# tinganchen/AlignQ

Hardware: AMD Instinct MI355X
Metric: images/sec (train step, CDF+ADMM) ResNet-20 8-bit (higher is better)
Workload: dtype f32; 1 GPU; resnet20 CIFAR-shape 3x32x32, 8W/8A CDF+ADMM full train step (cdf_alignment_admm/resnet-20-cifar-10), batch 128/GPU, HIP-graph replay, batch-norm folded into the site kernels, channels-last tensors, all Conv2d_Q convolutions on alignq_conv*_nhwc (exact-product bf16 MFMA); global_batch=128, parallelism=dp1

## Files before the change

alignq_amd/csrc/conv_kernels.hip:

```cpp
#include <hip/hip_runtime.h>
#include <stdint.h>
#include <stdlib.h>

#include "../../include/alignq.h"
#include "site_internal.h"
#include "wgrad_reduce_body.h"

namespace {

using namespace alignq_wgr;

typedef __bf16 bf16x8 __attribute__((ext_vector_type(8)));
typedef __bf16 bf16x4 __attribute__((ext_vector_type(4)));
typedef float f32x4 __attribute__((ext_vector_type(4)));
typedef short s16x4 __attribute__((ext_vector_type(4)));

__device__ __forceinline__ s16x4 tr_read(const __bf16* p) {
  return __builtin_amdgcn_ds_read_tr16_b64_v4i16((__attribute__((address_space(3))) s16x4*)(p));
}
__device__ __forceinline__ bf16x8 join8(s16x4 a, s16x4 b) {
  typedef short s16x8 __attribute__((ext_vector_type(8)));
  s16x8 v = {a[0], a[1], a[2], a[3], b[0], b[1], b[2], b[3]};
  return __builtin_bit_cast(bf16x8, v);
}


template <int xb>
__device__ __forceinline__ f32x4 fetch_act4(const float* __restrict__ x, int64_t off) {
  if constexpr (xb == 0) return *reinterpret_cast<const f32x4*>(x + off);
  if constexpr (xb == 2) {
    const s16x4 b = *reinterpret_cast<const s16x4*>(reinterpret_cast<const short*>(x) + off);
    return (f32x4){(float)b[0], (float)b[1], (float)b[2], (float)b[3]};
  }
  const char4 b = *reinterpret_cast<const char4*>(reinterpret_cast<const signed char*>(x) + off);
  return (f32x4){(float)b.x, (float)b.y, (float)b.z, (float)b.w};
}

struct BnLazy {
  const float* z;
  const float* ab;
  const float* save;
  const float* ktot;
  const float* part = nullptr;
  int n_tiles = 0, tile_f = 0;
  double inv_n = 1.0;
  float* dgamma = nullptr;
  float* dbeta = nullptr;
};

template <int C>
__device__ __forceinline__ void bn_totals_lds(const BnLazy& t, float* __restrict__ kt, bool publish) {
  static_assert(256 % C == 0, "thread -> (channel, group)");
  __shared__ double red[256][2];
  constexpr int G = 256 / C;
  const int tid = threadIdx.x;
  const int cp = C < t.tile_f ? C : t.tile_f;
  const int cyc = C / cp, cnt = t.n_tiles / cyc;
  const int c = tid % C, grp = tid / C;
  const int e = c % cp, t_first = c / cp;
  double s0 = 0, s1 = 0;
  constexpr int U = 16;
  for (int i0 = grp; i0 < cnt; i0 += G * U) {
    float2 v[U];
#pragma unroll
    for (int u = 0; u < U; u++) {
      const int i = i0 + u * G;
      const int ic = i < cnt ? i : cnt - 1;
      v[u] = *reinterpret_cast<const float2*>(t.part + ((int64_t)(ic * cyc + t_first) * cp + e) * 2);
// ... 11 lines not shown
#pragma unroll
    for (int g = 0; g < G; g++) { t0 += red[g * C + tid][0]; t1 += red[g * C + tid][1]; }
    kt[tid] = (float)(t0 * t.inv_n);
    kt[C + tid] = (float)(t1 * t.inv_n);
    if (publish) {
      if (t.dbeta) t.dbeta[tid] = (float)t0;
      if (t.dgamma) t.dgamma[tid] = (float)t1;
    }
  }
  __syncthreads();
}

__device__ __forceinline__ float4 bn_lazy4(const float4& g, const float4& z, const float4& a, const float4& m, const float4& is,
                                           const float4& k0, const float4& k1) {
  float4 o;
  o.x = a.x * (g.x - k0.x - (z.x - m.x) * is.x * k1.x);
  o.y = a.y * (g.y - k0.y - (z.y - m.y) * is.y * k1.y);
  o.z = a.z * (g.z - k0.z - (z.z - m.z) * is.z * k1.z);
  o.w = a.w * (g.w - k0.w - (z.w - m.w) * is.w * k1.w);
  return o;
}

template <int C> constexpr int conv_cp() { return C == 16 ? 16 : (C == 32 ? 48 : C + 8); }
template <int C, int WD, int PT>
struct ConvLds {
  static constexpr int kBf16 = 3 * ((PT / WD) + 2) * (WD + 2) * conv_cp<C>();
};

template <int C, int WD, int PT, bool DGRAD, int XB = 0>
__device__ __forceinline__ void conv3x3_body(const float* __restrict__ x, const float* __restrict__ w,
                                             float* __restrict__ y, int H, int total_rows, float nlev, __bf16* lds,
                                             int block, const float* __restrict__ add,
                                             float* __restrict__ bn_part = nullptr, int n_wg = 0,
                                             BnLazy lazy = BnLazy{nullptr, nullptr, nullptr, nullptr}, float xlev = 1.0f) {
  static_assert(XB == 0 || !DGRAD, "the data gradient reads fp32 dy");
  constexpr int xb = XB;
  constexpr int TR = PT / WD;
  constexpr int NS = (9 * C + 31) / 32;
  constexpr int NCG = C / 16;
  constexpr int NPP = 4 / NCG;
  constexpr int NG = PT / 16;
  constexpr int LW = WD + 2;
  constexpr int CP = conv_cp<C>();
  constexpr int LROWS = TR + 2;
  constexpr int ARR = LROWS * LW * CP;
  static_assert(3 * ARR == ConvLds<C, WD, PT>::kBf16, "LDS size");
  __bf16* Xhi = lds;
  __bf16* Xmi = lds + ARR;
  __bf16* Xlo = lds + 2 * ARR;

  const int tid = threadIdx.x, lane = tid & 63, wv = tid >> 6;
  const int row0 = block * TR;
  const int img_lo = (row0 / H) * H, img_hi = img_lo + H;
  {
    constexpr int C4 = C / 4;
    constexpr int N4 = LROWS * LW * C4;
    constexpr int NIT = (N4 + 255) / 256;
    float4 v[NIT];
#pragma unroll
    for (int it = 0; it < NIT; it++) {
      const int i = tid + 256 * it;
      const int c4 = i % C4, col = (i / C4) % LW, lr = i / (C4 * LW);
      const int grow = row0 + lr - 1;
      const bool ok = i < N4 && col >= 1 && col <= WD && grow >= img_lo && grow < img_hi && grow < total_rows;
      const int64_t off = ok ? ((int64_t)grow * WD + (col - 1)) * C + 4 * c4 : 0;
      const f32x4 ld = fetch_act4<XB>(x, off);
      v[it] = ok ? make_float4(ld[0], ld[1], ld[2], ld[3]) : make_float4(0.f, 0.f, 0.f, 0.f);
    }
    if (DGRAD && lazy.z) {
      float4 zz[NIT];
#pragma unroll
      for (int it = 0; it < NIT; it++) {
        const int i = tid + 256 * it;
        const int c4 = i % C4, col = (i / C4) % LW, lr = i / (C4 * LW);
        const int grow = row0 + lr - 1;
        const bool ok = i < N4 && col >= 1 && col <= WD && grow >= img_lo && grow < img_hi && grow < total_rows;
        zz[it] = *reinterpret_cast<const float4*>(lazy.z + (ok ? ((int64_t)grow * WD + (col - 1)) * C + 4 * c4 : 0));
      }
      const int c4t = tid % C4;
      const float4 a4 = *reinterpret_cast<const float4*>(lazy.ab + 4 * c4t);
      const float4 m4 = *reinterpret_cast<const float4*>(lazy.save + 4 * c4t);
      const float4 i4 = *reinterpret_cast<const float4*>(lazy.save + C + 4 * c4t);
      float4 k0, k1;
      if (lazy.part) {
        __shared__ __attribute__((aligned(16))) float kt[2 * C];
        bn_totals_lds<C>(lazy, kt, block == 0);
        k0 = *reinterpret_cast<const float4*>(kt + 4 * c4t);
        k1 = *reinterpret_cast<const float4*>(kt + C + 4 * c4t);
      } else {
        k0 = *reinterpret_cast<const float4*>(lazy.ktot + 4 * c4t);
        k1 = *reinterpret_cast<const float4*>(lazy.ktot + C + 4 * c4t);
      }
#pragma unroll
      for (int it = 0; it < NIT; it++) {
        const int i = tid + 256 * it;
        const int col = (i / C4) % LW, lr = i / (C4 * LW);
        const int grow = row0 + lr - 1;
        const bool ok = i < N4 && col >= 1 && col <= WD && grow >= img_lo && grow < img_hi && grow < total_rows;
        if (ok) v[it] = bn_lazy4(v[it], zz[it], a4, m4, i4, k0, k1);
      }
    }
#pragma unroll
    for (int it = 0; it < NIT; it++) {
      const int i = tid + 256 * it;
      if (i < N4) {
        const int c4 = i % C4, col = (i / C4) % LW, lr = i / (C4 * LW);
        bf16x4 h4, m4, l4;
        const float vv[4] = {v[it].x, v[it].y, v[it].z, v[it].w};
#pragma unroll
        for (int e = 0; e < 4; e++) {
          const __bf16 hi = (__bf16)vv[e];
          const float r1 = vv[e] - (float)hi;
          const __bf16 mi = (__bf16)r1;
          const float r2 = r1 - (float)mi;
          h4[e] = hi; m4[e] = mi; l4[e] = (__bf16)r2;
        }
        const int o = (lr * LW + col) * CP + 4 * c4;
        *reinterpret_cast<bf16x4*>(Xhi + o) = h4;
        *reinterpret_cast<bf16x4*>(Xmi + o) = m4;
        *reinterpret_cast<bf16x4*>(Xlo + o) = l4;
      }
    }
  }
  const int cog = wv % NCG, pp = wv / NCG;
  const int m = lane & 15, q = lane >> 4;
  bf16x8 ab[NS];
#pragma unroll
  for (int s = 0; s < NS; s++) {
    const int k0 = 32 * s + 8 * q;
    const int tap = k0 / C, c0 = k0 % C;
    float v[8];
    if (tap < 9) {
      if (!DGRAD) {
        const float* p = w + ((int64_t)(cog * 16 + m) * 9 + tap) * C + c0;
        const float4 a4 = *reinterpret_cast<const float4*>(p), b4 = *reinterpret_cast<const float4*>(p + 4);
        v[0] = a4.x; v[1] = a4.y; v[2] = a4.z; v[3] = a4.w; v[4] = b4.x; v[5] = b4.y; v[6] = b4.z; v[7] = b4.w;
      } else {
#pragma unroll
        for (int j = 0; j < 8; j++) v[j] = w[((int64_t)(c0 + j) * 9 + (8 - tap)) * C + cog * 16 + m];
      }
    } else {
#pragma unroll
      for (int j = 0; j < 8; j++) v[j] = 0.f;
    }
#pragma unroll
    for (int j = 0; j < 8; j++) ab[s][j] = (__bf16)rintf(v[j] * nlev);
  }
  __syncthreads();
  float bs[4] = {0.f, 0.f, 0.f, 0.f}, bq[4] = {0.f, 0.f, 0.f, 0.f};
  for (int g = pp; g < NG; g += NPP) {
    const int p = g * 16 + (lane & 15);
    const int r = p / WD, c = p % WD;
    f32x4 acc = {0.f, 0.f, 0.f, 0.f};
#pragma unroll
    for (int s = 0; s < NS; s++) {
      const int k0 = 32 * s + 8 * q;
      const int tap = k0 / C, c0 = k0 % C;
      bf16x8 bh, bm, bl;
      if (tap < 9) {
        const int ky = tap / 3, kx = tap % 3;
        const int o = ((r + ky) * LW + (c + kx)) * CP + c0;
        bh = *reinterpret_cast<const bf16x8*>(Xhi + o);
        bm = *reinterpret_cast<const bf16x8*>(Xmi + o);
        bl = *reinterpret_cast<const bf16x8*>(Xlo + o);
      } else {
#pragma unroll
        for (int j = 0; j < 8; j++) { bh[j] = (__bf16)0.f; bm[j] = (__bf16)0.f; bl[j] = (__bf16)0.f; }
      }
      if (DGRAD || xb == 0) acc = __builtin_amdgcn_mfma_f32_16x16x32_bf16(ab[s], bl, acc, 0, 0, 0);
      acc = __builtin_amdgcn_mfma_f32_16x16x32_bf16(ab[s], bm, acc, 0, 0, 0);
      acc = __builtin_amdgcn_mfma_f32_16x16x32_bf16(ab[s], bh, acc, 0, 0, 0);
    }
    const int grow = row0 + r;
    if (grow < total_rows) {
      const int64_t o = ((int64_t)grow * WD + c) * C + cog * 16 + 4 * q;
      const float den = (!DGRAD && xb != 0) ? nlev * xlev : nlev;
      float4 v = make_float4(acc[0] / den, acc[1] / den, acc[2] / den, acc[3] / den);
      if (add) {
        const float4 r = *reinterpret_cast<const float4*>(add + o);
        v.x += r.x; v.y += r.y; v.z += r.z; v.w += r.w;
      }
      *reinterpret_cast<float4*>(y + o) = v;
      bs[0] += v.x; bs[1] += v.y; bs[2] += v.z; bs[3] += v.w;
      bq[0] += v.x * v.x; bq[1] += v.y * v.y; bq[2] += v.z * v.z; bq[3] += v.w * v.w;
    }
  }
  if (!DGRAD && bn_part) {
    float* red = reinterpret_cast<float*>(lds);
#define ROW_SHR_ADD(V, CTRL) V += __builtin_bit_cast(float, __builtin_amdgcn_update_dpp(0, __builtin_bit_cast(int, V), CTRL, 0xf, 0xf, false))
#pragma unroll
    for (int e = 0; e < 4; e++) {
      ROW_SHR_ADD(bs[e], 0x111); ROW_SHR_ADD(bs[e], 0x112); ROW_SHR_ADD(bs[e], 0x114); ROW_SHR_ADD(bs[e], 0x118);
      ROW_SHR_ADD(bq[e], 0x111); ROW_SHR_ADD(bq[e], 0x112); ROW_SHR_ADD(bq[e], 0x114); ROW_SHR_ADD(bq[e], 0x118);
    }
#undef ROW_SHR_ADD
    __syncthreads();
    if ((lane & 15) == 15) {
#pragma unroll
      for (int e = 0; e < 4; e++) {
        red[(wv * 16 + 4 * q + e) * 2] = bs[e];
        red[(wv * 16 + 4 * q + e) * 2 + 1] = bq[e];
      }
    }
    __syncthreads();
    if (tid < C) {
      const int cg = tid / 16, cl = tid % 16;
      float s0 = 0.f, s1 = 0.f;
#pragma unroll
      for (int ppi = 0; ppi < NPP; ppi++) {
        const int w2 = ppi * NCG + cg;
        s0 += red[(w2 * 16 + cl) * 2];
        s1 += red[(w2 * 16 + cl) * 2 + 1];
      }
      bn_part[((int64_t)tid * n_wg + block) * 2] = s0;
      bn_part[((int64_t)tid * n_wg + block) * 2 + 1] = s1;
    }
  }
}

template <int C, int WD, int PT, bool DGRAD, int XB = 0>
__global__ __launch_bounds__(256) void conv3x3_nhwc_kernel(const float* __restrict__ x, const float* __restrict__ w,
                                                           float* __restrict__ y, int H, int total_rows, float nlev,
                                                           const float* __restrict__ add, float* __restrict__ bn_part,
                                                           float xlev) {
  __shared__ __attribute__((aligned(16))) __bf16 lds[ConvLds<C, WD, PT>::kBf16];
  conv3x3_body<C, WD, PT, DGRAD, XB>(x, w, y, H, total_rows, nlev, lds, blockIdx.x, add, bn_part, gridDim.x,
                                     BnLazy{nullptr, nullptr, nullptr, nullptr}, xlev);
}

template <int CIN, int COUT, int WDI, int KS, int S, int PT>
struct ConvGen {
  static constexpr int WDO = WDI / S, TR = PT / WDO;
  static constexpr int LROWS = KS == 3 ? TR * S + (S == 1 ? 2 : 1) : TR;
  static constexpr int LW = KS == 3 ? WDI + 2 : WDO;
  static constexpr int CP = CIN + 8;
  static constexpr int ARR = LROWS * LW * CP;
};

template <int CIN, int COUT, int WDI, int KS, int S, int PT>
__device__ __forceinline__ void convgen_fwd_body(const float* __restrict__ x, const float* __restrict__ w,
                                                 float* __restrict__ y, int H, int total_rows, float nlev,
                                                 float* __restrict__ bn_part, __bf16* lds, int block, int n_wg) {
  using G = ConvGen<CIN, COUT, WDI, KS, S, PT>;
  constexpr int WDO = G::WDO, TR = G::TR, LROWS = G::LROWS, LW = G::LW, CP = G::CP, ARR = G::ARR;
  constexpr int NS = (KS * KS * CIN + 31) / 32;
  constexpr int NCG = COUT / 16, NPP = 4 / NCG, NG = PT / 16;
  static_assert(NCG == 1 || NCG == 2 || NCG == 4, "output channels");
  __bf16* Xhi = lds;
  __bf16* Xmi = lds + ARR;
  __bf16* Xlo = lds + 2 * ARR;
  const int tid = threadIdx.x, lane = tid & 63, wv = tid >> 6;
  const int row0 = block * TR;
  const int Hin = H * S;
  const int img_lo = (row0 / H) * Hin, img_hi = img_lo + Hin;
  {
    constexpr int C4 = CIN / 4;
    constexpr int N4 = LROWS * LW * C4;
    constexpr int NIT = (N4 + 255) / 256;
    float4 v[NIT];
#pragma unroll
    for (int it = 0; it < NIT; it++) {
      const int i = tid + 256 * it;
      const int c4 = i % C4, col = (i / C4) % LW, lr = i / (C4 * LW);
      int grow, gcol;
      if (KS == 3) { grow = row0 * S - 1 + lr; gcol = col - 1; }
      else { grow = (row0 + lr) * S; gcol = col * S; }
      const bool ok = i < N4 && gcol >= 0 && gcol < WDI && grow >= img_lo && grow < img_hi;
      v[it] = *reinterpret_cast<const float4*>(x + (ok ? ((int64_t)grow * WDI + gcol) * CIN + 4 * c4 : 0));
      if (!ok) v[it] = make_float4(0.f, 0.f, 0.f, 0.f);
    }
#pragma unroll
    for (int it = 0; it < NIT; it++) {
      const int i = tid + 256 * it;
      if (i < N4) {
        const int c4 = i % C4, col = (i / C4) % LW, lr = i / (C4 * LW);
        bf16x4 h4, m4, l4;
        const float vv[4] = {v[it].x, v[it].y, v[it].z, v[it].w};
#pragma unroll
        for (int e = 0; e < 4; e++) {
          const __bf16 hi = (__bf16)vv[e];
          const float r1 = vv[e] - (float)hi;
          const __bf16 mi = (__bf16)r1;
          h4[e] = hi; m4[e] = mi; l4[e] = (__bf16)(r1 - (float)mi);
        }
        const int o = (lr * LW + col) * CP + 4 * c4;
        *reinterpret_cast<bf16x4*>(Xhi + o) = h4;
        *reinterpret_cast<bf16x4*>(Xmi + o) = m4;
        *reinterpret_cast<bf16x4*>(Xlo + o) = l4;
      }
    }
  }
  const int cog = wv % NCG, pp = wv / NCG;
  const int m = lane & 15, q = lane >> 4;
  bf16x8 ab[NS];
#pragma unroll
  for (int s = 0; s < NS; s++) {
    const int k0 = 32 * s + 8 * q;
    const int tap = k0 / CIN, c0 = k0 % CIN;
    if (tap < KS * KS) {
      const float* p = w + ((int64_t)(cog * 16 + m) * (KS * KS) + tap) * CIN + c0;
      const float4 a4 = *reinterpret_cast<const float4*>(p), b4 = *reinterpret_cast<const float4*>(p + 4);
      const float v[8] = {a4.x, a4.y, a4.z, a4.w, b4.x, b4.y, b4.z, b4.w};
#pragma unroll
      for (int j = 0; j < 8; j++) ab[s][j] = (__bf16)rintf(v[j] * nlev);
    } else {
#pragma unroll
      for (int j = 0; j < 8; j++) ab[s][j] = (__bf16)0.f;
    }
  }
  __syncthreads();
  float bs[4] = {0.f, 0.f, 0.f, 0.f}, bq[4] = {0.f, 0.f, 0.f, 0.f};
  for (int g = pp; g < NG; g += NPP) {
    const int p = g * 16 + (lane & 15);
    const int r = p / WDO, c = p % WDO;
    f32x4 acc = {0.f, 0.f, 0.f, 0.f};
#pragma unroll
    for (int s = 0; s < NS; s++) {
      const int k0 = 32 * s + 8 * q;
      const int tap = k0 / CIN, c0 = k0 % CIN;
      bf16x8 bh, bm, bl;
      if (tap < KS * KS) {
        const int ky = tap / KS, kx = tap % KS;
        const int o = (KS == 3 ? ((r * S + ky) * LW + (c * S + kx)) : (r * LW + c)) * CP + c0;
        bh = *reinterpret_cast<const bf16x8*>(Xhi + o);
        bm = *reinterpret_cast<const bf16x8*>(Xmi + o);
        bl = *reinterpret_cast<const bf16x8*>(Xlo + o);
      } else {
#pragma unroll
        for (int j = 0; j < 8; j++) { bh[j] = (__bf16)0.f; bm[j] = (__bf16)0.f; bl[j] = (__bf16)0.f; }
      }
      acc = __builtin_amdgcn_mfma_f32_16x16x32_bf16(ab[s], bl, acc, 0, 0, 0);
      acc = __builtin_amdgcn_mfma_f32_16x16x32_bf16(ab[s], bm, acc, 0, 0, 0);
      acc = __builtin_amdgcn_mfma_f32_16x16x32_bf16(ab[s], bh, acc, 0, 0, 0);
    }
    const int grow = row0 + r;
    if (grow < total_rows) {
      const float4 v = make_float4(acc[0] / nlev, acc[1] / nlev, acc[2] / nlev, acc[3] / nlev);
      *reinterpret_cast<float4*>(y + ((int64_t)grow * WDO + c) * COUT + cog * 16 + 4 * q) = v;
      bs[0] += v.x; bs[1] += v.y; bs[2] += v.z; bs[3] += v.w;
      bq[0] += v.x * v.x; bq[1] += v.y * v.y; bq[2] += v.z * v.z; bq[3] += v.w * v.w;
    }
  }
  if (bn_part) {
    float* red = reinterpret_cast<float*>(lds);
#define ROW_SHR_ADD(V, CTRL) V += __builtin_bit_cast(float, __builtin_amdgcn_update_dpp(0, __builtin_bit_cast(int, V), CTRL, 0xf, 0xf, false))
#pragma unroll
    for (int e = 0; e < 4; e++) {
      ROW_SHR_ADD(bs[e], 0x111); ROW_SHR_ADD(bs[e], 0x112); ROW_SHR_ADD(bs[e], 0x114); ROW_SHR_ADD(bs[e], 0x118);
      ROW_SHR_ADD(bq[e], 0x111); ROW_SHR_ADD(bq[e], 0x112); ROW_SHR_ADD(bq[e], 0x114); ROW_SHR_ADD(bq[e], 0x118);
    }
#undef ROW_SHR_ADD
    __syncthreads();
    if ((lane & 15) == 15) {
#pragma unroll
      for (int e = 0; e < 4; e++) {
        red[(wv * 16 + 4 * q + e) * 2] = bs[e];
        red[(wv * 16 + 4 * q + e) * 2 + 1] = bq[e];
      }
    }
    __syncthreads();
    if (tid < COUT) {
      const int cg = tid / 16, cl = tid % 16;
      float s0 = 0.f, s1 = 0.f;
#pragma unroll
      for (int ppi = 0; ppi < NPP; ppi++) {
        s0 += red[((ppi * NCG + cg) * 16 + cl) * 2];
        s1 += red[((ppi * NCG + cg) * 16 + cl) * 2 + 1];
      }
      bn_part[((int64_t)tid * n_wg + block) * 2] = s0;
      bn_part[((int64_t)tid * n_wg + block) * 2 + 1] = s1;
    }
  }
}

template <int CIN, int COUT, int WDI, int KS, int S, int PT>
__global__ __launch_bounds__(256) void convgen_fwd_kernel(const float* __restrict__ x, const float* __restrict__ w,
                                                          float* __restrict__ y, int H, int total_rows, float nlev,
                                                          float* __restrict__ bn_part) {
  __shared__ __attribute__((aligned(16))) __bf16 lds[3 * ConvGen<CIN, COUT, WDI, KS, S, PT>::ARR];
  convgen_fwd_body<CIN, COUT, WDI, KS, S, PT>(x, w, y, H, total_rows, nlev, bn_part, lds, blockIdx.x, gridDim.x);
}

template <int CIN, int COUT, int WDI, int PT3, int PT1>
__global__ __launch_bounds__(256) void transition_fwd_kernel(const float* __restrict__ x, const float* __restrict__ w3,
                                                             const float* __restrict__ w1, float* __restrict__ y3,
                                                             float* __restrict__ y1, int H, int total_rows, float nlev,
                                                             float* __restrict__ part3, float* __restrict__ part1, int n3) {
  constexpr int A3 = ConvGen<CIN, COUT, WDI, 3, 2, PT3>::ARR, A1 = ConvGen<CIN, COUT, WDI, 1, 2, PT1>::ARR;
  __shared__ __attribute__((aligned(16))) __bf16 lds[3 * (A3 > A1 ? A3 : A1)];
  if ((int)blockIdx.x < n3)
// ... 415 lines not shown
  return e == hipSuccess ? 0 : (int)e;
}

template <int C, int WD, int PT>
int launch(const float* x, const float* w, float* y, int B, int H, int dgrad, float nlev, const float* add, float* bn_part,
           hipStream_t st, int xb = 0, float xlev = 1.0f) {
  constexpr int TR = PT / WD;
  const int total_rows = B * H;
  if (H % TR) return ALIGNQ_EUNSUPPORTED;
  const int grid = total_rows / TR;
  if (dgrad) hipLaunchKernelGGL((conv3x3_nhwc_kernel<C, WD, PT, true, 0>), grid, 256, 0, st, x, w, y, H, total_rows, nlev, add, nullptr, 1.0f);
  else if (xb == 2) hipLaunchKernelGGL((conv3x3_nhwc_kernel<C, WD, PT, false, 2>), grid, 256, 0, st, x, w, y, H, total_rows, nlev, add, bn_part, xlev);
  else if (xb == 1) hipLaunchKernelGGL((conv3x3_nhwc_kernel<C, WD, PT, false, 1>), grid, 256, 0, st, x, w, y, H, total_rows, nlev, add, bn_part, xlev);
  else hipLaunchKernelGGL((conv3x3_nhwc_kernel<C, WD, PT, false, 0>), grid, 256, 0, st, x, w, y, H, total_rows, nlev, add, bn_part, xlev);
  hipError_t e = hipGetLastError();
  return e == hipSuccess ? 0 : (int)e;
}

typedef float f32x16 __attribute__((ext_vector_type(16)));

template <int CIN, int COUT, int WDI, int KS, int S, int PT>
struct WgradGeo {
  static constexpr int WDO = WDI / S, TR = PT / WDO, NT = KS * KS;
  static constexpr int CB = (CIN < COUT ? CIN : COUT) >= 32 ? 32 : 16;
  static constexpr int XROWS = KS == 3 ? TR * S + (S == 1 ? 2 : 1) : TR;
  static constexpr int LW = KS == 3 ? WDI + 2 : WDO;
  static constexpr int XA = XROWS * LW * CB;
  static constexpr int DA = PT * CB;
  static constexpr int kRed = 3 * NT * 4 * 64 * 4;
  static constexpr int kBytes = (3 * (XA + DA) * 2) > kRed ? (3 * (XA + DA) * 2) : kRed;
  static constexpr int kFloats = kBytes / 4;
};
template <int C, int WD, int PT>
struct WgradLds : WgradGeo<C, C, WD, 3, 1, PT> {};

template <int CIN, int COUT, int WDI, int KS, int S, int PT, int XB = 0>
__device__ __forceinline__ void wgrad_body(const float* __restrict__ x, const float* __restrict__ dy,
                                           float* __restrict__ slabs, int H, int n_tiles, float* lds_f, int bx, int gx,
                                           int by, BnLazy lazy = BnLazy{nullptr, nullptr, nullptr, nullptr}, float xlev = 1.0f) {
  constexpr int xb = XB;
  using G = WgradGeo<CIN, COUT, WDI, KS, S, PT>;
  constexpr int WDO = G::WDO, TR = G::TR, NT = G::NT, CB = G::CB, LW = G::LW, XA = G::XA, DA = G::DA, XROWS = G::XROWS;
  constexpr int NBLK = CIN / CB;
  constexpr int NSTEP = PT / 32;
  static_assert(WDO % 8 == 0 && PT % 32 == 0, "a lane group's 8 pixels lie in one output row");
  __bf16* lds = reinterpret_cast<__bf16*>(lds_f);
  __bf16* Xi[3] = {lds, lds + XA, lds + 2 * XA};
  __bf16* Di[3] = {lds + 3 * XA, lds + 3 * XA + DA, lds + 3 * XA + 2 * DA};
  const int tid = threadIdx.x, lane = tid & 63, wv = tid >> 6;
  const int bi = by / NBLK, bj = by % NBLK;
  const int cob = CB == 32 ? (wv >> 1) : 0, cib = CB == 32 ? (wv & 1) : 0;
  const int g = lane >> 4, q = (lane & 15) >> 2, pcol = 4 * (lane & 3);

  f32x4 acc[NT];
#pragma unroll
  for (int t = 0; t < NT; t++) acc[t] = (f32x4){0.f, 0.f, 0.f, 0.f};

  constexpr int C4 = CB / 4;
  constexpr int N4 = XROWS * LW * C4;
  constexpr int M4 = PT * C4;
  constexpr int NIX = (N4 + 255) / 256, NID = (M4 + 255) / 256;
  f32x4 rx[NIX], rd[NID], rz[NID];
  const int per = (n_tiles + gx - 1) / gx;
  const int t_begin = bx * per, t_end = (t_begin + per < n_tiles) ? t_begin + per : n_tiles;
  int nxt = t_begin;
  if (nxt < t_end) {
    const int row0_ = nxt * TR;
    const int img_lo_ = (row0_ / H) * (H * S), img_hi_ = img_lo_ + H * S;
#pragma unroll
    for (int it = 0; it < NIX; it++) {
      const int i = tid + 256 * it;
      const int c4 = i % C4, col = (i / C4) % LW, lr = i / (C4 * LW);
      const int grow = KS == 3 ? row0_ * S - 1 + lr : (row0_ + lr) * S;
      const int gcol = KS == 3 ? col - 1 : col * S;
      const bool ok = i < N4 && gcol >= 0 && gcol < WDI && grow >= img_lo_ && grow < img_hi_;
      const int64_t off = ok ? ((int64_t)grow * WDI + gcol) * CIN + bj * CB + 4 * c4 : 0;
      rx[it] = fetch_act4<XB>(x, off);
      if (!ok) rx[it] = (f32x4){0.f, 0.f, 0.f, 0.f};
    }
#pragma unroll
    for (int it = 0; it < NID; it++) {
      const int i = tid + 256 * it;
      const int64_t off = i < M4 ? ((int64_t)row0_ * WDO + i / C4) * COUT + bi * CB + 4 * (i % C4) : 0;
      rd[it] = *reinterpret_cast<const f32x4*>(dy + off);
      if (lazy.z) rz[it] = *reinterpret_cast<const f32x4*>(lazy.z + off);
    }
  }
  f32x4 la = {0, 0, 0, 0}, lm = la, li = la, lk0 = la, lk1 = la;
  if (lazy.z) {
    const int cq = bi * CB + 4 * (tid % C4);
    la = *reinterpret_cast<const f32x4*>(lazy.ab + cq);
    lm = *reinterpret_cast<const f32x4*>(lazy.save + cq);
    li = *reinterpret_cast<const f32x4*>(lazy.save + COUT + cq);
    if (lazy.part) {
      __shared__ __attribute__((aligned(16))) float kt[2 * COUT];
      bn_totals_lds<COUT>(lazy, kt, false);
      lk0 = *reinterpret_cast<const f32x4*>(kt + cq);
      lk1 = *reinterpret_cast<const f32x4*>(kt + COUT + cq);
    } else {
      lk0 = *reinterpret_cast<const f32x4*>(lazy.ktot + cq);
      lk1 = *reinterpret_cast<const f32x4*>(lazy.ktot + COUT + cq);
    }
  }
  for (int tile = t_begin; tile < t_end; tile++) {
    __syncthreads();
#pragma unroll
    for (int it = 0; it < NIX; it++) {
      const int i = tid + 256 * it;
      if (i < N4) {
        const int c4 = i % C4, col = (i / C4) % LW, lr = i / (C4 * LW);
        bf16x4 h4, m4, l4;
#pragma unroll
        for (int e = 0; e < 4; e++) {
          const float v = rx[it][e];
          const __bf16 hi = (__bf16)v;
          const float r1 = v - (float)hi;
          const __bf16 mi = (__bf16)r1;
          h4[e] = hi; m4[e] = mi; l4[e] = (__bf16)(r1 - (float)mi);
        }
        const int o = (lr * LW + col) * CB + 4 * c4;
        *reinterpret_cast<bf16x4*>(Xi[0] + o) = h4;
        *reinterpret_cast<bf16x4*>(Xi[1] + o) = m4;
        *reinterpret_cast<bf16x4*>(Xi[2] + o) = l4;
      }
    }
#pragma unroll
    for (int it = 0; it < NID; it++) {
      const int i = tid + 256 * it;
      if (i < M4) {
        bf16x4 h4, m4, l4;
        f32x4 dv = rd[it];
        if (lazy.z) dv = la * (dv - lk0 - (rz[it] - lm) * li * lk1);
#pragma unroll
        for (int e = 0; e < 4; e++) {
          const float v = dv[e];
          const __bf16 hi = (__bf16)v;
          const float r1 = v - (float)hi;
          const __bf16 mi = (__bf16)r1;
          h4[e] = hi; m4[e] = mi; l4[e] = (__bf16)(r1 - (float)mi);
        }
        const int o = (i / C4) * CB + 4 * (i % C4);
        *reinterpret_cast<bf16x4*>(Di[0] + o) = h4;
        *reinterpret_cast<bf16x4*>(Di[1] + o) = m4;
        *reinterpret_cast<bf16x4*>(Di[2] + o) = l4;
      }
    }
    __syncthreads();
    nxt = tile + 1;
    if (nxt < t_end) {
      const int row0_ = nxt * TR;
      const int img_lo_ = (row0_ / H) * (H * S), img_hi_ = img_lo_ + H * S;
#pragma unroll
      for (int it = 0; it < NIX; it++) {
        const int i = tid + 256 * it;
        const int c4 = i % C4, col = (i / C4) % LW, lr = i / (C4 * LW);
        const int grow = KS == 3 ? row0_ * S - 1 + lr : (row0_ + lr) * S;
        const int gcol = KS == 3 ? col - 1 : col * S;
        const bool ok = i < N4 && gcol >= 0 && gcol < WDI && grow >= img_lo_ && grow < img_hi_;
        const int64_t off = ok ? ((int64_t)grow * WDI + gcol) * CIN + bj * CB + 4 * c4 : 0;
        rx[it] = fetch_act4<XB>(x, off);
        if (!ok) rx[it] = (f32x4){0.f, 0.f, 0.f, 0.f};
      }
#pragma unroll
      for (int it = 0; it < NID; it++) {
        const int i = tid + 256 * it;
        const int64_t off = i < M4 ? ((int64_t)row0_ * WDO + i / C4) * COUT + bi * CB + 4 * (i % C4) : 0;
        rd[it] = *reinterpret_cast<const f32x4*>(dy + off);
        if (lazy.z) rz[it] = *reinterpret_cast<const f32x4*>(lazy.z + off);
      }
    }
    for (int s = (CB == 16 ? wv : 0); s < NSTEP; s += (CB == 16 ? 4 : 1)) {
      const int p0 = 32 * s + 8 * g;
      const int r = p0 / WDO, c0 = p0 % WDO;
      bf16x8 a[3];
#pragma unroll
      for (int t = 0; t < 3; t++) {
        const __bf16* pa = Di[t] + (p0 + q) * CB + cob * 16 + pcol;
        a[t] = join8(tr_read(pa), tr_read(pa + 4 * CB));
      }
#pragma unroll
      for (int tap = 0; tap < NT; tap++) {
        const int ky = tap / KS, kx = tap % KS;
        bf16x8 b[3];
#pragma unroll
        for (int t = 0; t < 3; t++) {
          const __bf16* pb = Xi[t] + (KS == 3 ? ((r * S + ky) * LW + ((c0 + q) * S + kx)) : (r * LW + c0 + q)) * CB +
                             cib * 16 + pcol;
          b[t] = join8(tr_read(pb), tr_read(pb + 4 * (KS == 3 ? S : 1) * CB));
        }
        f32x4 v = acc[tap];
        v = __builtin_amdgcn_mfma_f32_16x16x32_bf16(a[1], b[1], v, 0, 0, 0);
        if (xb == 0) v = __builtin_amdgcn_mfma_f32_16x16x32_bf16(a[0], b[2], v, 0, 0, 0);
        v = __builtin_amdgcn_mfma_f32_16x16x32_bf16(a[2], b[0], v, 0, 0, 0);
        v = __builtin_amdgcn_mfma_f32_16x16x32_bf16(a[0], b[1], v, 0, 0, 0);
        v = __builtin_amdgcn_mfma_f32_16x16x32_bf16(a[1], b[0], v, 0, 0, 0);
        v = __builtin_amdgcn_mfma_f32_16x16x32_bf16(a[0], b[0], v, 0, 0, 0);
        acc[tap] = v;
      }
    }
  }
  float* slab = slabs + (int64_t)bx * (NT * CIN * COUT);
  if (xb != 0) {
    const float inv = 1.0f / xlev;
#pragma unroll
    for (int t = 0; t < NT; t++) acc[t] = acc[t] * inv;
  }
  if (CB == 16) {
    float* red = lds_f;
    __syncthreads();
    if (wv > 0) {
#pragma unroll
      for (int t = 0; t < NT; t++)
#pragma unroll
        for (int e = 0; e < 4; e++) red[(((wv - 1) * NT + t) * 4 + e) * 64 + lane] = acc[t][e];
    }
    __syncthreads();
    if (wv == 0) {
#pragma unroll
      for (int t = 0; t < NT; t++) {
#pragma unroll
        for (int e = 0; e < 4; e++) {
          float v = acc[t][e];
#pragma unroll
          for (int w2 = 0; w2 < 3; w2++) v += red[((w2 * NT + t) * 4 + e) * 64 + lane];
          __builtin_nontemporal_store(v, &slab[((int64_t)(bi * CB + 4 * (lane >> 4) + e) * NT + t) * CIN + bj * CB + (lane & 15)]);
        }
      }
    }
  } else {
#pragma unroll
    for (int t = 0; t < NT; t++)
#pragma unroll
      for (int e = 0; e < 4; e++)
        __builtin_nontemporal_store(acc[t][e], &slab[((int64_t)(bi * CB + cob * 16 + 4 * (lane >> 4) + e) * NT + t) * CIN + bj * CB + cib * 16 + (lane & 15)]);
  }
}

template <int C, int WD, int PT, int XB = 0>
__device__ __forceinline__ void wgrad3x3_body(const float* __restrict__ x, const float* __restrict__ dy,
                                              float* __restrict__ slabs, int H, int n_tiles, float* lds_f, int bx, int gx,
                                              int by, BnLazy lazy = BnLazy{nullptr, nullptr, nullptr, nullptr}, float xlev = 1.0f) {
  wgrad_body<C, C, WD, 3, 1, PT, XB>(x, dy, slabs, H, n_tiles, lds_f, bx, gx, by, lazy, xlev);
}

template <int CIN, int COUT, int WDI, int KS, int S, int PT>
__global__ __launch_bounds__(256) void wgradgen_kernel(const float* __restrict__ x, const float* __restrict__ dy,
                                                       float* __restrict__ slabs, int H, int n_tiles, BnLazy lazy) {
  __shared__ __attribute__((aligned(16))) float lds[WgradGeo<CIN, COUT, WDI, KS, S, PT>::kFloats];
  wgrad_body<CIN, COUT, WDI, KS, S, PT>(x, dy, slabs, H, n_tiles, lds, blockIdx.x, gridDim.x, blockIdx.y, lazy);
}

template <int C, int WD, int PT, int XB>
__global__ __launch_bounds__(256) void wgrad3x3_nhwc_kernel(const float* __restrict__ x, const float* __restrict__ dy,
                                                            float* __restrict__ slabs, int H, int n_tiles, float xlev) {
  __shared__ __attribute__((aligned(16))) float lds[WgradLds<C, WD, PT>::kFloats];
  wgrad3x3_body<C, WD, PT, XB>(x, dy, slabs, H, n_tiles, lds, blockIdx.x, gridDim.x, blockIdx.y,
                               BnLazy{nullptr, nullptr, nullptr, nullptr}, xlev);
}

template <int C, int WD, int PTD, int PTW, int XB>
__global__ __launch_bounds__(256) void conv3x3_bwd_kernel(const float* __restrict__ x, const float* __restrict__ dy,
                                                          const float* __restrict__ w, float* __restrict__ dx,
                                                          float* __restrict__ slabs, int H, int total_rows, float nlev,
                                                          int n_tiles_w, int splits, int nblk2,
                                                          const float* __restrict__ add, BnLazy lazy, float xlev, int dg_R,
                                                          RedFill fill, int n_dg) {
  constexpr int kBytesD = ConvLds<C, WD, PTD>::kBf16 * 2, kBytesW = WgradLds<C, WD, PTW>::kFloats * 4;
  static_assert(kBytesD >= 4096 || kBytesW >= 4096, "the filler role's 4 KB");
  __shared__ __attribute__((aligned(16))) unsigned char lds[kBytesD > kBytesW ? kBytesD : kBytesW];
  const int n_wg = splits * nblk2;
  if ((int)blockIdx.x < n_wg) {
    wgrad3x3_body<C, WD, PTW, XB>(x, dy, slabs, H, n_tiles_w, reinterpret_cast<float*>(lds), blockIdx.x % splits, splits,
                                  blockIdx.x / splits, lazy, xlev);
  } else if ((int)blockIdx.x >= n_wg + n_dg) {
    const int fb = blockIdx.x - n_wg - n_dg;
    int it = 0;
    while (it + 1 < kFill && fb >= fill.blk0[it + 1]) it++;
    wgrad_reduce_body<256>(fill.slabs[it], fill.n_slabs[it], fill.n_elem[it], fill.dw[it], fb - fill.blk0[it],
                           reinterpret_cast<float*>(lds));
  } else {
    int m = blockIdx.x - n_wg;
    if (dg_R > 0) {
      const int i = (m / (8 * dg_R)) * 8 + (m & 7), r = (m >> 3) % dg_R;
      m = dg_R * i + r;
    }
    conv3x3_body<C, WD, PTD, true>(dy, w, dx, H, total_rows, nlev, reinterpret_cast<__bf16*>(lds), m, add, nullptr, 0, lazy);
  }
}

template <int CIN, int COUT, int WDI, int PTW3, int PTW1, int PTD>
__global__ __launch_bounds__(256) void transition_bwd_kernel(const float* __restrict__ x, const float* __restrict__ dy3,
                                                             const float* __restrict__ dy1, const float* __restrict__ w3,
                                                             const float* __restrict__ w1, float* __restrict__ dx,
                                                             float* __restrict__ slabs3, float* __restrict__ slabs1, int Ho,
                                                             int n_tiles3, int n_tiles1, int splits3, int splits1, int n_d,
                                                             float nlev, const float* __restrict__ add, BnLazy lazy3,
                                                             BnLazy lazy1, int dg_R) {
  using G3 = WgradGeo<CIN, COUT, WDI, 3, 2, PTW3>;
  using G1 = WgradGeo<CIN, COUT, WDI, 1, 2, PTW1>;
  constexpr int NBY = (COUT / G3::CB) * (CIN / G3::CB);
  static_assert(G3::CB == G1::CB, "same channel blocking");
  constexpr int kD = DgradS2Lds<CIN, COUT, WDI, 3, PTD, true>::kBf16 * 2;
  constexpr int kW = G3::kBytes > G1::kBytes ? G3::kBytes : G1::kBytes;
  __shared__ __attribute__((aligned(16))) unsigned char lds[kD > kW ? kD : kW];
  const int n_w3 = splits3 * NBY;
  const int b = blockIdx.x;
  if (b < n_d) {
    int m = b;
    if (dg_R > 0) {
      const int i = (m / (8 * dg_R)) * 8 + (m & 7), r = (m >> 3) % dg_R;
      m = dg_R * i + r;
    }
    dgrad_s2_body<CIN, COUT, WDI, 3, PTD, true>(dy3, w3, dx, 2 * Ho, 0x7fffffff, nlev, add, lazy3,
                                                reinterpret_cast<__bf16*>(lds), m, dy1, w1, lazy1);
  } else if (b < n_d + n_w3) {
    const int c = b - n_d;
    wgrad_body<CIN, COUT, WDI, 3, 2, PTW3>(x, dy3, slabs3, Ho, n_tiles3, reinterpret_cast<float*>(lds), c % splits3, splits3,
                                           c / splits3, lazy3);
  } else {
    const int c = b - n_d - n_w3;
    wgrad_body<CIN, COUT, WDI, 1, 2, PTW1>(x, dy1, slabs1, Ho, n_tiles1, reinterpret_cast<float*>(lds), c % splits1, splits1,
                                           c / splits1, lazy1);
  }
}

__global__ __launch_bounds__(1024) void wgrad_reduce_kernel(const float* __restrict__ slabs, int n_slabs, int n_elem,
                                                            float* __restrict__ dw) {
  __shared__ __attribute__((aligned(16))) float part[4096];
  wgrad_reduce_body(slabs, n_slabs, n_elem, dw, blockIdx.x, part);
}

constexpr int kWgMulti = 32;
struct WgChunk {
  const float* slabs[kWgMulti];
  float* dw[kWgMulti];
  int n_slabs[kWgMulti];
  int n_elem[kWgMulti];
  int blk0[kWgMulti + 1];
};
__global__ __launch_bounds__(1024) void wgrad_reduce_multi_kernel(WgChunk c, int cnt) {
// ... 341 lines not shown
      !alignq_conv_gen_bn_parts(B, H_in, W_in, CIN, COUT, 1, 2))
    return ALIGNQ_EUNSUPPORTED;
  if ((reinterpret_cast<uintptr_t>(x) | reinterpret_cast<uintptr_t>(dy3) | reinterpret_cast<uintptr_t>(dy1) |
       reinterpret_cast<uintptr_t>(wt3) | reinterpret_cast<uintptr_t>(wt1) | reinterpret_cast<uintptr_t>(dx) |
       reinterpret_cast<uintptr_t>(add)) & 15)
    return ALIGNQ_EUNSUPPORTED;
  hipStream_t st = (hipStream_t)stream;
  const float nlev = (float)((1 << w_bit) - 1);
  BnLazy lazy3{bn3_z, bn3_ab, bn3_save, bn3_ktot}, lazy1{bn1_z, bn1_ab, bn1_save, bn1_ktot};
  const int HWo = (H_in / 2) * (W_in / 2);
  if (int rc = lazy_parts(lazy3, bn3_dx_part, bn3_dgamma, bn3_dbeta, B, COUT, HWo)) return rc;
  if (int rc = lazy_parts(lazy1, bn1_dx_part, bn1_dgamma, bn1_dbeta, B, COUT, HWo)) return rc;
  const int Ho = H_in / 2;
  if (CIN == 16)
    return launch_transition_bwd<16, 32, 32, 64, 128, 256>(x, dy3, dy1, wt3, wt1, dx, (float*)ws3, (float*)ws1, B, Ho, nlev,
                                                          n_slabs3, n_slabs1, add, lazy3, lazy1, st);
  if (CIN == 32)
    return launch_transition_bwd<32, 64, 16, 64, 64, 128>(x, dy3, dy1, wt3, wt1, dx, (float*)ws3, (float*)ws1, B, Ho, nlev,
                                                         n_slabs3, n_slabs1, add, lazy3, lazy1, st);
  return ALIGNQ_EUNSUPPORTED;
}

int alignq_conv_stem_bn_parts(int B, int H, int W) { return (W == 32 && B >= 1 && H >= 4 && H % 4 == 0) ? B * H / 4 : 0; }
int alignq_conv_stem_nhwc_fwd(const float* x, const float* wt, float* y, int B, int H, int W, int w_bit, float* bn_part,
                              void* stream) {
  if (!x || !wt || !y) return ALIGNQ_EINVAL;
  if (w_bit < 1 || w_bit > 8 || !alignq_conv_stem_bn_parts(B, H, W)) return ALIGNQ_EUNSUPPORTED;
  if (reinterpret_cast<uintptr_t>(y) & 15) return ALIGNQ_EUNSUPPORTED;
  hipLaunchKernelGGL(stem_fwd_kernel, B * H / 4, 256, 0, (hipStream_t)stream, x, wt, y, H, B * H, (float)((1 << w_bit) - 1),
                     bn_part);
  hipError_t e = hipGetLastError();
  return e == hipSuccess ? 0 : (int)e;
}
int alignq_conv_stem_nhwc_wgrad(const float* x, const float* dy, float* dw, void* ws, int B, int H, int W, int* n_slabs_out,
                                const float* bn_z, const float* bn_ab, const float* bn_save, const float* bn_ktot,
                                const float* bn_dx_part, float* bn_dgamma, float* bn_dbeta, void* stream) {
  if (!x || !dy || !ws || (!dw && !n_slabs_out)) return ALIGNQ_EINVAL;
  if (bn_z && (!bn_ab || !bn_save || (!bn_ktot && !bn_dx_part))) return ALIGNQ_EINVAL;
  if (!alignq_conv_stem_bn_parts(B, H, W) || (reinterpret_cast<uintptr_t>(dy) & 15)) return ALIGNQ_EUNSUPPORTED;
  hipStream_t st = (hipStream_t)stream;
  const int n_tiles = B * H / 4;
  const int splits = n_tiles < 256 ? n_tiles : 256;
  BnLazy lazy{bn_z, bn_ab, bn_save, bn_ktot};
  if (int rc = lazy_parts(lazy, bn_dx_part, bn_dgamma, bn_dbeta, B, 16, H * W)) return rc;
  hipLaunchKernelGGL(stem_wgrad_kernel, splits, 256, 0, st, x, dy, (float*)ws, H, n_tiles, lazy);
  hipError_t e = hipGetLastError();
  if (e != hipSuccess) return (int)e;
  if (n_slabs_out) { *n_slabs_out = splits; return 0; }
  hipLaunchKernelGGL(wgrad_reduce_kernel, wgrad_reduce_blocks(splits, 16 * 27), 1024, 0, st, (const float*)ws, splits, 16 * 27, dw);
  e = hipGetLastError();
  return e == hipSuccess ? 0 : (int)e;
}

}
```

Baseline: 126,900 images/sec.

## Software-pipeline LDS loads against MFMAs across pixel groups in conv bodies

Restructures the conv3x3 and strided conv inner loops so each wave keeps accumulators for all of its pixel groups and double-buffers the hi/mid/lo LDS fragments, issuing the next slice's loads before the current slice's MFMAs, with a sched_barrier between them. The dgrad path is limited to batches of two groups. Weight quantisation moves inside the activation-staging scope and replaces the tap branch with a clamped tap plus mask. It also skips the lo-part MFMA load when it is unused, and adds a waves_per_eu hint on the backward kernel. The intent is to hide LDS latency and raise MFMA issue density, at the cost of more VGPRs and possibly lower occupancy. Timing stamps compiled out by default are added too.

```diff
diff --git a/alignq_amd/csrc/conv_kernels.hip b/alignq_amd/csrc/conv_kernels.hip
--- a/alignq_amd/csrc/conv_kernels.hip
+++ b/alignq_amd/csrc/conv_kernels.hip
@@ -14,6 +14,22 @@
 typedef __bf16 bf16x4 __attribute__((ext_vector_type(4)));
 typedef float f32x4 __attribute__((ext_vector_type(4)));
 typedef short s16x4 __attribute__((ext_vector_type(4)));
+
+#ifdef ALIGNQ_STAMPS
+__device__ unsigned long long g_conv_stamps[64];
+__device__ unsigned long long g_conv_blk[2][4096];
+#define STAMP(on, i)                                                          \
+  do {                                                                        \
+    if ((on) && threadIdx.x == 0) g_conv_stamps[i] = wall_clock64();          \
+  } while (0)
+#define BSTAMP(which)                                                                          \
+  do {                                                                                         \
+    if (threadIdx.x == 0 && blockIdx.x < 4096) g_conv_blk[which][blockIdx.x] = wall_clock64(); \
+  } while (0)
+#else
+#define STAMP(on, i) do { } while (0)
+#define BSTAMP(which) do { } while (0)
+#endif
 
 __device__ __forceinline__ s16x4 tr_read(const __bf16* p) {
   return __builtin_amdgcn_ds_read_tr16_b64_v4i16((__attribute__((address_space(3))) s16x4*)(p));
@@ -131,6 +147,11 @@
   const int tid = threadIdx.x, lane = tid & 63, wv = tid >> 6;
   const int row0 = block * TR;
   const int img_lo = (row0 / H) * H, img_hi = img_lo + H;
+  [[maybe_unused]] constexpr int SB = DGRAD ? 8 : 0;
+  STAMP(block == 0, SB + 0);
+  const int cog = wv % NCG, pp = wv / NCG;
+  const int m = lane & 15, q = lane >> 4;
+  bf16x8 ab[NS];
   {
     constexpr int C4 = C / 4;
     constexpr int N4 = LROWS * LW * C4;
@@ -146,6 +167,7 @@
       const f32x4 ld = fetch_act4<XB>(x, off);
       v[it] = ok ? make_float4(ld[0], ld[1], ld[2], ld[3]) : make_float4(0.f, 0.f, 0.f, 0.f);
     }
+    STAMP(block == 0, SB + 1);
     if (DGRAD && lazy.z) {
       float4 zz[NIT];
 #pragma unroll
@@ -200,61 +222,84 @@
         *reinterpret_cast<bf16x4*>(Xlo + o) = l4;
       }
     }
-  }
-  const int cog = wv % NCG, pp = wv / NCG;
-  const int m = lane & 15, q = lane >> 4;
-  bf16x8 ab[NS];
-#pragma unroll
-  for (int s = 0; s < NS; s++) {
-    const int k0 = 32 * s + 8 * q;
-    const int tap = k0 / C, c0 = k0 % C;
-    float v[8];
-    if (tap < 9) {
+    STAMP(block == 0, SB + 2);
+#pragma unroll
+    for (int s = 0; s < NS; s++) {
+      const int k0 = 32 * s + 8 * q;
+      const bool live = k0 / C < 9;
+      const int tap = live ? k0 / C : 8, c0 = k0 % C;
+      float wr[8];
       if (!DGRAD) {
         const float* p = w + ((int64_t)(cog * 16 + m) * 9 + tap) * C + c0;
         const float4 a4 = *reinterpret_cast<const float4*>(p), b4 = *reinterpret_cast<const float4*>(p + 4);
-        v[0] = a4.x; v[1] = a4.y; v[2] = a4.z; v[3] = a4.w; v[4] = b4.x; v[5] = b4.y; v[6] = b4.z; v[7] = b4.w;
+        wr[0] = a4.x; wr[1] = a4.y; wr[2] = a4.z; wr[3] = a4.w; wr[4] = b4.x; wr[5] = b4.y; wr[6] = b4.z; wr[7] = b4.w;
       } else {
 #pragma unroll
-        for (int j = 0; j < 8; j++) v[j] = w[((int64_t)(c0 + j) * 9 + (8 - tap)) * C + cog * 16 + m];
-      }
-    } else {
-#pragma unroll
-      for (int j = 0; j < 8; j++) v[j] = 0.f;
-    }
-#pragma unroll
-    for (int j = 0; j < 8; j++) ab[s][j] = (__bf16)rintf(v[j] * nlev);
+        for (int j = 0; j < 8; j++) wr[j] = w[((int64_t)(c0 + j) * 9 + (8 - tap)) * C + cog * 16 + m];
+      }
+#pragma unroll
+      for (int j = 0; j < 8; j++) ab[s][j] = (__bf16)rintf((live ? wr[j] : 0.f) * nlev);
+    }
+    STAMP(block == 0, SB + 3);
   }
   __syncthreads();
+  constexpr int GW = NG / NPP;
+  static_assert(NG % NPP == 0, "every wave takes the same number of pixel groups");
+  int bo[GW];
+  f32x4 acc[GW];
+#pragma unroll
+  for (int gi = 0; gi < GW; gi++) {
+    const int p = (pp + gi * NPP) * 16 + (lane & 15);
+    bo[gi] = ((p / WD) * LW + (p % WD)) * CP;
+    acc[gi] = (f32x4){0.f, 0.f, 0.f, 0.f};
+  }
+  constexpr int GB = (DGRAD && GW > 2) ? 2 : GW;
+  static_assert(GW % GB == 0, "whole batches of groups");
+#pragma unroll
+  for (int g0 = 0; g0 < GW; g0 += GB) {
+    bf16x8 bh[2][GB], bm[2][GB], bl[2][GB];
+#pragma unroll
+    for (int s = 0; s <= NS; s++) {
+      if (s < NS) {
+        const int k0 = 32 * s + 8 * q;
+        const bool live = k0 / C < 9;
+        const int tap = live ? k0 / C : 8, c0 = k0 % C;
+        const int to = ((tap / 3) * LW + (tap % 3)) * CP + c0;
+#pragma unroll
+        for (int gi = 0; gi < GB; gi++) {
+          const int o = bo[g0 + gi] + to;
+          bh[s & 1][gi] = *reinterpret_cast<const bf16x8*>(Xhi + o);
+          bm[s & 1][gi] = *reinterpret_cast<const bf16x8*>(Xmi + o);
+          if (DGRAD || xb == 0) bl[s & 1][gi] = *reinterpret_cast<const bf16x8*>(Xlo + o);
+          if ((9 * C) % 32 != 0 && !live) {
+#pragma unroll
+            for (int j = 0; j < 8; j++) { bh[s & 1][gi][j] = (__bf16)0.f; bm[s & 1][gi][j] = (__bf16)0.f; bl[s & 1][gi][j] = (__bf16)0.f; }
+          }
+        }
+      }
+      __builtin_amdgcn_sched_barrier(0);
+      if (s > 0) {
+        const int u = s - 1;
+#pragma unroll
+        for (int gi = 0; gi < GB; gi++) {
+          f32x4 a = acc[g0 + gi];
+          if (DGRAD || xb == 0) a = __builtin_amdgcn_mfma_f32_16x16x32_bf16(ab[u], bl[u & 1][gi], a, 0, 0, 0);
+          a = __builtin_amdgcn_mfma_f32_16x16x32_bf16(ab[u], bm[u & 1][gi], a, 0, 0, 0);
+          acc[g0 + gi] = __builtin_amdgcn_mfma_f32_16x16x32_bf16(ab[u], bh[u & 1][gi], a, 0, 0, 0);
+        }
+      }
+    }
+  }
   float bs[4] = {0.f, 0.f, 0.f, 0.f}, bq[4] = {0.f, 0.f, 0.f, 0.f};
-  for (int g = pp; g < NG; g += NPP) {
-    const int p = g * 16 + (lane & 15);
+#pragma unroll
+  for (int gi = 0; gi < GW; gi++) {
+    const int p = (pp + gi * NPP) * 16 + (lane & 15);
     const int r = p / WD, c = p % WD;
-    f32x4 acc = {0.f, 0.f, 0.f, 0.f};
-#pragma unroll
-    for (int s = 0; s < NS; s++) {
-      const int k0 = 32 * s + 8 * q;
-      const int tap = k0 / C, c0 = k0 % C;
-      bf16x8 bh, bm, bl;
-      if (tap < 9) {
-        const int ky = tap / 3, kx = tap % 3;
-        const int o = ((r + ky) * LW + (c + kx)) * CP + c0;
-        bh = *reinterpret_cast<const bf16x8*>(Xhi + o);
-        bm = *reinterpret_cast<const bf16x8*>(Xmi + o);
-        bl = *reinterpret_cast<const bf16x8*>(Xlo + o);
-      } else {
-#pragma unroll
-        for (int j = 0; j < 8; j++) { bh[j] = (__bf16)0.f; bm[j] = (__bf16)0.f; bl[j] = (__bf16)0.f; }
-      }
-      if (DGRAD || xb == 0) acc = __builtin_amdgcn_mfma_f32_16x16x32_bf16(ab[s], bl, acc, 0, 0, 0);
-      acc = __builtin_amdgcn_mfma_f32_16x16x32_bf16(ab[s], bm, acc, 0, 0, 0);
-      acc = __builtin_amdgcn_mfma_f32_16x16x32_bf16(ab[s], bh, acc, 0, 0, 0);
-    }
     const int grow = row0 + r;
     if (grow < total_rows) {
       const int64_t o = ((int64_t)grow * WD + c) * C + cog * 16 + 4 * q;
       const float den = (!DGRAD && xb != 0) ? nlev * xlev : nlev;
-      float4 v = make_float4(acc[0] / den, acc[1] / den, acc[2] / den, acc[3] / den);
+      float4 v = make_float4(acc[gi][0] / den, acc[gi][1] / den, acc[gi][2] / den, acc[gi][3] / den);
       if (add) {
         const float4 r = *reinterpret_cast<const float4*>(add + o);
         v.x += r.x; v.y += r.y; v.z += r.z; v.w += r.w;
@@ -264,6 +309,7 @@
       bq[0] += v.x * v.x; bq[1] += v.y * v.y; bq[2] += v.z * v.z; bq[3] += v.w * v.w;
     }
   }
+  STAMP(block == 0, SB + 4);
   if (!DGRAD && bn_part) {
     float* red = reinterpret_cast<float*>(lds);
 #define ROW_SHR_ADD(V, CTRL) V += __builtin_bit_cast(float, __builtin_amdgcn_update_dpp(0, __builtin_bit_cast(int, V), CTRL, 0xf, 0xf, false))
@@ -295,6 +341,7 @@
       bn_part[((int64_t)tid * n_wg + block) * 2 + 1] = s1;
     }
   }
+  STAMP(block == 0, SB + 5);
 }
 
 template <int C, int WD, int PT, bool DGRAD, int XB = 0>
@@ -332,6 +379,9 @@
   const int row0 = block * TR;
   const int Hin = H * S;
   const int img_lo = (row0 / H) * Hin, img_hi = img_lo + Hin;
+  const int cog = wv % NCG, pp = wv / NCG;
+  const int m = lane & 15, q = lane >> 4;
+  bf16x8 ab[NS];
   {
     constexpr int C4 = CIN / 4;
     constexpr int N4 = LROWS * LW * C4;
@@ -368,53 +418,70 @@
         *reinterpret_cast<bf16x4*>(Xlo + o) = l4;
       }
     }
-  }
-  const int cog = wv % NCG, pp = wv / NCG;
-  const int m = lane & 15, q = lane >> 4;
-  bf16x8 ab[NS];
-#pragma unroll
-  for (int s = 0; s < NS; s++) {
-    const int k0 = 32 * s + 8 * q;
-    const int tap = k0 / CIN, c0 = k0 % CIN;
-    if (tap < KS * KS) {
+#pragma unroll
+    for (int s = 0; s < NS; s++) {
+      const int k0 = 32 * s + 8 * q;
+      const bool live = k0 / CIN < KS * KS;
+      const int tap = live ? k0 / CIN : KS * KS - 1, c0 = k0 % CIN;
       const float* p = w + ((int64_t)(cog * 16 + m) * (KS * KS) + tap) * CIN + c0;
       const float4 a4 = *reinterpret_cast<const float4*>(p), b4 = *reinterpret_cast<const float4*>(p + 4);
-      const float v[8] = {a4.x, a4.y, a4.z, a4.w, b4.x, b4.y, b4.z, b4.w};
-#pragma unroll
-      for (int j = 0; j < 8; j++) ab[s][j] = (__bf16)rintf(v[j] * nlev);
-    } else {
-#pragma unroll
-      for (int j = 0; j < 8; j++) ab[s][j] = (__bf16)0.f;
+      const float wr[8] = {a4.x, a4.y, a4.z, a4.w, b4.x, b4.y, b4.z, b4.w};
+#pragma unroll
+      for (int j = 0; j < 8; j++) ab[s][j] = (__bf16)rintf((live ? wr[j] : 0.f) * nlev);
     }
   }
   __syncthreads();
+  constexpr int GW = NG / NPP;
+  static_assert(NG % NPP == 0, "every wave takes the same number of pixel groups");
+  int bo[GW];
+  f32x4 acc[GW];
+#pragma unroll
+  for (int gi = 0; gi < GW; gi++) {
+    const int p = (pp + gi * NPP) * 16 + (lane & 15);
+    const int r = p / WDO, c = p % WDO;
+    bo[gi] = (KS == 3 ? (r * S * LW + c * S) : (r * LW + c)) * CP;
+    acc[gi] = (f32x4){0.f, 0.f, 0.f, 0.f};
+  }
+  bf16x8 bh[2][GW], bm[2][GW], bl[2][GW];
+#pragma unroll
+  for (int s = 0; s <= NS; s++) {
+    if (s < NS) {
+      const int k0 = 32 * s + 8 * q;
+      const bool live = k0 / CIN < KS * KS;
+      const int tap = live ? k0 / CIN : KS * KS - 1, c0 = k0 % CIN;
+      const int to = (KS == 3 ? ((tap / KS) * LW + (tap % KS)) * CP : 0) + c0;
+#pragma unroll
+      for (int gi = 0; gi < GW; gi++) {
+        const int o = bo[gi] + to;
+        bh[s & 1][gi] = *reinterpret_cast<const bf16x8*>(Xhi + o);
+        bm[s & 1][gi] = *reinterpret_cast<const bf16x8*>(Xmi + o);
+        bl[s & 1][gi] = *reinterpret_cast<const bf16x8*>(Xlo + o);
+        if ((KS * KS * CIN) % 32 != 0 && !live) {
+#pragma unroll
+          for (int j = 0; j < 8; j++) { bh[s & 1][gi][j] = (__bf16)0.f; bm[s & 1][gi][j] = (__bf16)0.f; bl[s & 1][gi][j] = (__bf16)0.f; }
+        }
+      }
+    }
+    __builtin_amdgcn_sched_barrier(0);
+    if (s > 0) {
+      const int u = s - 1;
+#pragma unroll
+      for (int gi = 0; gi < GW; gi++) {
+        f32x4 a = acc[gi];
+        a = __builtin_amdgcn_mfma_f32_16x16x32_bf16(ab[u], bl[u & 1][gi], a, 0, 0, 0);
+        a = __builtin_amdgcn_mfma_f32_16x16x32_bf16(ab[u], bm[u & 1][gi], a, 0, 0, 0);
+        acc[gi] = __builtin_amdgcn_mfma_f32_16x16x32_bf16(ab[u], bh[u & 1][gi], a, 0, 0, 0);
+      }
+    }
+  }
   float bs[4] = {0.f, 0.f, 0.f, 0.f}, bq[4] = {0.f, 0.f, 0.f, 0.f};
-  for (int g = pp; g < NG; g += NPP) {
-    const int p = g * 16 + (lane & 15);
+#pragma unroll
+  for (int gi = 0; gi < GW; gi++) {
+    const int p = (pp + gi * NPP) * 16 + (lane & 15);
     const int r = p / WDO, c = p % WDO;
-    f32x4 acc = {0.f, 0.f, 0.f, 0.f};
-#pragma unroll
-    for (int s = 0; s < NS; s++) {
-      const int k0 = 32 * s + 8 * q;
-      const int tap = k0 / CIN, c0 = k0 % CIN;
-      bf16x8 bh, bm, bl;
-      if (tap < KS * KS) {
-        const int ky = tap / KS, kx = tap % KS;
-        const int o = (KS == 3 ? ((r * S + ky) * LW + (c * S + kx)) : (r * LW + c)) * CP + c0;
-        bh = *reinterpret_cast<const bf16x8*>(Xhi + o);
-        bm = *reinterpret_cast<const bf16x8*>(Xmi + o);
-        bl = *reinterpret_cast<const bf16x8*>(Xlo + o);
-      } else {
-#pragma unroll
-        for (int j = 0; j < 8; j++) { bh[j] = (__bf16)0.f; bm[j] = (__bf16)0.f; bl[j] = (__bf16)0.f; }
-      }
-      acc = __builtin_amdgcn_mfma_f32_16x16x32_bf16(ab[s], bl, acc, 0, 0, 0);
-      acc = __builtin_amdgcn_mfma_f32_16x16x32_bf16(ab[s], bm, acc, 0, 0, 0);
-      acc = __builtin_amdgcn_mfma_f32_16x16x32_bf16(ab[s], bh, acc, 0, 0, 0);
-    }
     const int grow = row0 + r;
     if (grow < total_rows) {
-      const float4 v = make_float4(acc[0] / nlev, acc[1] / nlev, acc[2] / nlev, acc[3] / nlev);
+      const float4 v = make_float4(acc[gi][0] / nlev, acc[gi][1] / nlev, acc[gi][2] / nlev, acc[gi][3] / nlev);
       *reinterpret_cast<float4*>(y + ((int64_t)grow * WDO + c) * COUT + cog * 16 + 4 * q) = v;
       bs[0] += v.x; bs[1] += v.y; bs[2] += v.z; bs[3] += v.w;
       bq[0] += v.x * v.x; bq[1] += v.y * v.y; bq[2] += v.z * v.z; bq[3] += v.w * v.w;
@@ -936,6 +1003,8 @@
   const int cob = CB == 32 ? (wv >> 1) : 0, cib = CB == 32 ? (wv & 1) : 0;
   const int g = lane >> 4, q = (lane & 15) >> 2, pcol = 4 * (lane & 3);
 
+  [[maybe_unused]] const bool st_on = bx == 0 && by == 0;
+  STAMP(st_on, 16);
   f32x4 acc[NT];
 #pragma unroll
   for (int t = 0; t < NT; t++) acc[t] = (f32x4){0.f, 0.f, 0.f, 0.f};
@@ -986,6 +1055,7 @@
       lk1 = *reinterpret_cast<const f32x4*>(lazy.ktot + COUT + cq);
     }
   }
+  STAMP(st_on, 17);
   for (int tile = t_begin; tile < t_end; tile++) {
     __syncthreads();
 #pragma unroll
@@ -1030,6 +1100,7 @@
       }
     }
     __syncthreads();
+    STAMP(st_on && tile - t_begin < 16, 18 + 2 * (tile - t_begin));
     nxt = tile + 1;
     if (nxt < t_end) {
       const int row0_ = nxt * TR;
@@ -1082,7 +1153,9 @@
         acc[tap] = v;
       }
     }
-  }
+    STAMP(st_on && tile - t_begin < 16, 19 + 2 * (tile - t_begin));
+  }
+  STAMP(st_on, 50);
   float* slab = slabs + (int64_t)bx * (NT * CIN * COUT);
   if (xb != 0) {
     const float inv = 1.0f / xlev;
@@ -1118,6 +1191,7 @@
       for (int e = 0; e < 4; e++)
         __builtin_nontemporal_store(acc[t][e], &slab[((int64_t)(bi * CB + cob * 16 + 4 * (lane >> 4) + e) * NT + t) * CIN + bj * CB + cib * 16 + (lane & 15)]);
   }
+  STAMP(st_on, 51);
 }
 
 template <int C, int WD, int PT, int XB = 0>
@@ -1143,7 +1217,8 @@
 }
 
 template <int C, int WD, int PTD, int PTW, int XB>
-__global__ __launch_bounds__(256) void conv3x3_bwd_kernel(const float* __restrict__ x, const float* __restrict__ dy,
+__global__ __launch_bounds__(256) __attribute__((amdgpu_waves_per_eu(C == 16 ? 3 : 2, C == 16 ? 3 : 8)))
+void conv3x3_bwd_kernel(const float* __restrict__ x, const float* __restrict__ dy,
                                                           const float* __restrict__ w, float* __restrict__ dx,
                                                           float* __restrict__ slabs, int H, int total_rows, float nlev,
                                                           int n_tiles_w, int splits, int nblk2,
@@ -1153,6 +1228,7 @@
   static_assert(kBytesD >= 4096 || kBytesW >= 4096, "the filler role's 4 KB");
   __shared__ __attribute__((aligned(16))) unsigned char lds[kBytesD > kBytesW ? kBytesD : kBytesW];
   const int n_wg = splits * nblk2;
+  BSTAMP(0);
   if ((int)blockIdx.x < n_wg) {
     wgrad3x3_body<C, WD, PTW, XB>(x, dy, slabs, H, n_tiles_w, reinterpret_cast<float*>(lds), blockIdx.x % splits, splits,
                                   blockIdx.x / splits, lazy, xlev);
@@ -1170,6 +1246,7 @@
     }
     conv3x3_body<C, WD, PTD, true>(dy, w, dx, H, total_rows, nlev, reinterpret_cast<__bf16*>(lds), m, add, nullptr, 0, lazy);
   }
+  BSTAMP(1);
 }
 
 template <int CIN, int COUT, int WDI, int PTW3, int PTW1, int PTD>
@@ -1617,4 +1694,13 @@
   return e == hipSuccess ? 0 : (int)e;
 }
 
-}
+#ifdef ALIGNQ_STAMPS
+int alignq_debug_read_conv_stamps(unsigned long long* host_out) {
+  return (int)hipMemcpyFromSymbol(host_out, HIP_SYMBOL(g_conv_stamps), sizeof(unsigned long long) * 64);
+}
+int alignq_debug_read_conv_block_stamps(unsigned long long* host_out) {
+  return (int)hipMemcpyFromSymbol(host_out, HIP_SYMBOL(g_conv_blk), sizeof(unsigned long long) * 2 * 4096);
+}
+#endif
+
+}
```

Measured after the change: 130,500 images/sec, median of 6. +2.9%, better.
